# David-OConnor/molchanica

Hardware: AMD Instinct MI355X
Metric: MD atom-updates/sec (and steps/sec), 1M-atom solvated box (higher is better)
Workload: dtype f32

## Files before the change

### include/mdx.h

```cpp
#ifndef MDX_H
#define MDX_H

#include <stddef.h>
#include <stdint.h>

#ifdef __cplusplus
extern "C" {
#endif

#define MDX_OK       0
#define MDX_EPARAM  (-1)
#define MDX_EDEVICE (-2)
#define MDX_ENAN    (-3)
#define MDX_EOOM    (-4)

#define MDX_OVR_BONDED_DISABLED           0x1u
#define MDX_OVR_COULOMB_DISABLED          0x2u
#define MDX_OVR_LJ_DISABLED               0x4u
#define MDX_OVR_LONG_RANGE_RECIP_DISABLED 0x8u

#define MDX_ATOM_STATIC      0x1u
#define MDX_ATOM_BONDED_ONLY 0x2u
#define MDX_ATOM_GHOST       0x4u

// ... 122 lines not shown

int mdx_device_count(void);

const char* mdx_last_error(void);

void mdx_config_default(mdx_config* cfg);

int mdx_create(const mdx_system* sys, const mdx_config* cfg, int device, mdx_handle** out);
void mdx_destroy(mdx_handle* h);

int mdx_step(mdx_handle* h, float dt, const float* ext_forces, uint32_t n_steps);

int      mdx_set_position_restraints(mdx_handle* h, uint32_t n, const uint32_t* idx, const float* ref, const float* k,
                                     const float* flat_bottom);
uint32_t mdx_position_restraints_read(mdx_handle* h, uint32_t capacity, uint32_t* idx, float* ref, float* k, float* flat_bottom);
int      mdx_restraint_energy(mdx_handle* h, double* energy, double* virial);

int mdx_energy(mdx_handle* h, mdx_energies* out);

int mdx_single_point(const mdx_system* sys, const mdx_config* cfg, int device,
                     mdx_energies* out, float* forces_or_null);
void mdx_single_point_release(void);

int mdx_download(mdx_handle* h, int which, float* dst );
int mdx_upload(mdx_handle* h, int which, const float* src );
int mdx_upload_range(mdx_handle* h, int which, uint32_t first, uint32_t count, const float* src );

int mdx_set_box(mdx_handle* h, const float lo[3], const float hi[3]);
int mdx_rebuild_spatial_caches(mdx_handle* h);

uint64_t mdx_step_count(const mdx_handle* h);

int mdx_neighbor_list(mdx_handle* h, uint32_t* offsets , uint32_t* idx );

enum { MDX_HC_FLEXIBLE = 0, MDX_HC_SHAKE = 1, MDX_HC_LINEAR = 2 };
int mdx_set_hydrogen_constraint(mdx_handle* h, int kind, uint32_t lincs_order, uint32_t lincs_iter, float shake_tolerance);
const char* mdx_constraint_description(mdx_handle* h);

int mdx_profile(mdx_handle* h, int enable);
int mdx_get_stats(mdx_handle* h, mdx_stats* out);
int mdx_pair_launch_info(const mdx_handle* h, uint32_t out[24]);
int mdx_pair_body_info(const mdx_handle* h, uint32_t out[4]);
int mdx_fused_triad_info(const mdx_handle* h, uint32_t out[4]);
int mdx_get_skin(const mdx_handle* h, float* skin, int* tuning);

#define MDX_THERMOSTAT_NONE      0
#define MDX_THERMOSTAT_BERENDSEN 1
#define MDX_THERMOSTAT_CSVR      2

#define MDX_INTEGRATOR_VERLET_VELOCITY 0
#define MDX_INTEGRATOR_LEAPFROG        1
#define MDX_INTEGRATOR_LANGEVIN_MIDDLE 2
int mdx_set_integrator(mdx_handle* h, int kind, float gamma_per_ps, float temperature, uint64_t seed);

int mdx_set_alchemical_softcore(mdx_handle* h, float alpha, float sigma_min);
int mdx_configure_alchemical_window(mdx_handle* h, uint32_t mol_index, double lambda);

#define MDX_MAX_FOREIGN_LAMBDAS 32
int      mdx_set_foreign_lambdas(mdx_handle* h, uint32_t n, const double* lambdas);
int      mdx_foreign_energies(mdx_handle* h, double* du , uint32_t n);
uint32_t mdx_snapshot_foreign_count(const mdx_handle* h, uint32_t k);
int      mdx_snapshot_read_foreign(mdx_handle* h, uint32_t k, double* du, uint32_t n);

#define MDX_BAROSTAT_NONE      0
#define MDX_BAROSTAT_BERENDSEN 1
#define MDX_BAR_PER_KCAL_MOL_A3 69476.95
// ... 174 lines not shown
```

### molchanica_amd/csrc/mdx_api.hip

```cpp
#include "mdx_comm.h"
#include <algorithm>
#include <atomic>
#include <chrono>
#include <cfloat>
#include <cmath>
#include <cstring>
#include <dlfcn.h>
#include <mutex>
#include <unordered_map>

static thread_local std::string g_last_error;
void mdx_set_error(const std::string& s) { g_last_error = s; }

static inline unsigned div_up(unsigned a, unsigned b) { return (a + b - 1) / b; }
static bool cut_on(float rc) { return rc > 0.f && std::isfinite(rc); }
static uint32_t f2u(float f) { uint32_t u; std::memcpy(&u, &f, 4); return u; }
static float u2f(uint32_t u) { float f; std::memcpy(&f, &u, 4); return f; }

#define FAIL(code, msg) do { mdx_set_error(msg); return (code); } while (0)

template <typename T>
static int upload_vec(T** dptr, const std::vector<T>& v, hipStream_t st) {
    if (*dptr) { (void)hipFree(*dptr); *dptr = nullptr; }
    HIP_TRY(hipMalloc((void**)dptr, std::max<size_t>(sizeof(T) * v.size(), 16)));
// ... 1526 lines not shown
                              h->d.slot_of, h->d.posq, (float4*)d_out4,
                              flag_word >= 0 ? &h->d.ctl->disp2[flag_word] : nullptr);
    HIP_TRY(hipGetLastError());
    return MDX_OK;
}

extern "C" int mdx_unpack_positions(mdx_handle* h, const uint32_t* d_gid, uint32_t n, const float* d_in4,
                                    const float* d_shift4, int32_t flag_word) {
    if (!h || (n && (!d_gid || !d_in4)) || flag_word > (int32_t)MDX_MAX_CHUNK + 1) FAIL(MDX_EPARAM, "bad argument");
    if (!h->in_slot_space) FAIL(MDX_EPARAM, "spatial caches not built");
    const bool dual = h->dual_on && h->chunk_s >= 0;
    if (n) hipLaunchKernelGGL(unpack_pos_kernel, dim3(div_up(n, 256)), dim3(256), 0, h->stream, n, d_gid,
                              h->d.slot_of, h->d.posq, (const float4*)d_in4, (const float4*)d_shift4,
                              flag_word >= 0 ? &h->d.ctl->disp2[flag_word] : nullptr,
                              dual ? h->d.ref : nullptr,
                              dual ? (mdx_dd_split_now(h) ? &h->d.ctl->prune_ghost[h->chunk_s + 1]
                                                                                                      : &h->d.ctl->prune[h->chunk_s + 1]) : nullptr,
                              0.5f * h->inner_skin * (1.0f - 1.0e-4f),
                              h->dd ? h->box_hi[0] - h->box_lo[0] : 0.f, h->dd ? h->box_hi[1] - h->box_lo[1] : 0.f,
                              h->dd ? h->box_hi[2] - h->box_lo[2] : 0.f, (dual && h->path_split) ? h->d.path : nullptr);
    HIP_TRY(hipGetLastError());
    h->forces_valid = false;
    if (!dual) h->moved_outside = true;
    return MDX_OK;
}

extern "C" void* mdx_stream(mdx_handle* h) { return h ? (void*)h->stream : nullptr; }
extern "C" int mdx_debug_half_stats(mdx_handle* h, unsigned long long out[6]) {
    HIP_TRY(hipStreamSynchronize(h->stream));
    HIP_TRY(hipMemcpy(out, h->d.inner_count + MDX_EPART, sizeof(unsigned long long) * 6, hipMemcpyDeviceToHost));
    return MDX_OK;
}

static int posre_install(mdx_handle* h) {
    DeviceState& d = h->d;
    hipStream_t st = h->stream;
    const uint32_t N = h->N, R_old = h->n_roles, n = h->n_posre;
    std::vector<uint32_t> off_old(N + 1);
    std::vector<RoleRec> rec_old(R_old);
    std::vector<float4> prm(h->n_prm_base);
    HIP_TRY(hipMemcpyAsync(off_old.data(), d.role_off_o, sizeof(uint32_t) * (N + 1), hipMemcpyDeviceToHost, st));
    if (R_old) HIP_TRY(hipMemcpyAsync(rec_old.data(), d.role_rec_o, sizeof(RoleRec) * R_old, hipMemcpyDeviceToHost, st));
    if (!prm.empty()) HIP_TRY(hipMemcpyAsync(prm.data(), d.role_prm, sizeof(float4) * prm.size(), hipMemcpyDeviceToHost, st));
    HIP_TRY(hipStreamSynchronize(st));
    if ((size_t)h->n_prm_base + n >= ((size_t)1 << 24)) FAIL(MDX_EPARAM, "more than 16.7 M distinct bonded parameter sets with the restraints");
    std::vector<uint32_t> which(N, MDX_INVALID);
    for (uint32_t k = 0; k < n; ++k) which[h->posre_idx[k]] = k;
    std::vector<uint32_t> off(N + 1, 0);
    std::vector<RoleRec> rec;
    rec.reserve((size_t)R_old + n);
    for (uint32_t i = 0; i < N; ++i) {
        for (uint32_t k = off_old[i]; k < off_old[i + 1]; ++k)
            if ((rec_old[k].meta & 0xFu) != ROLE_POSRE) rec.push_back(rec_old[k]);
        if (which[i] != MDX_INVALID) {
            const uint32_t k = which[i];
            RoleRec r{};
            r.p[0] = i; r.p[1] = 0u; r.p[2] = f2u(h->posre_b[k]);
            r.meta = ROLE_POSRE | ((h->n_prm_base + k) << 8);
            rec.push_back(r);
        }
        off[i + 1] = (uint32_t)rec.size();
    }
    for (uint32_t k = 0; k < n; ++k)
        prm.push_back(make_float4(h->posre_ref[3 * k], h->posre_ref[3 * k + 1], h->posre_ref[3 * k + 2], h->posre_k[k]));
    const uint32_t R = (uint32_t)rec.size();
    h->n_roles = R;
// ... 77 lines not shown
```

### molchanica_amd/csrc/mdx_grid.hip

```cpp
#include "mdx_internal.h"
#include <atomic>
#include <chrono>
#include <algorithm>
#include <cfloat>
#include <cmath>

#define WAVE_LDS_SYNC()                                      \
    do {                                                     \
        __builtin_amdgcn_fence(__ATOMIC_SEQ_CST, "workgroup"); \
        __builtin_amdgcn_wave_barrier();                     \
    } while (0)

static inline unsigned div_up(unsigned a, unsigned b) { return (a + b - 1) / b; }

constexpr int SCAN_THREADS = 256;
constexpr int SCAN_ITEMS = 8;
constexpr int SCAN_TILE = SCAN_THREADS * SCAN_ITEMS;

template <int THREADS>
__device__ __forceinline__ uint32_t block_exclusive_scan(uint32_t v, uint32_t* s_wave , uint32_t* total) {
    const int lane = threadIdx.x & 63, wave = threadIdx.x >> 6;
    uint32_t inc = v;
#pragma unroll
    for (int d = 1; d < 64; d <<= 1) {
// ... 745 lines not shown
                const uint32_t sp = spc[q];
                if (sp == MDX_INVALID) continue;
#pragma unroll
                for (int e = 0; e < 8; ++e)
                    if (jcs[e] == (sp >> 3)) m &= ~(1ull << (8 * e + (sp & 7)));
            }
            for (uint32_t k = eb + LB_SPC; k < ee; ++k) {
                uint32_t sp = a.slot_of[a.excl_idx[k]];
                if (sp == MDX_INVALID) continue;
#pragma unroll
                for (int e = 0; e < 8; ++e)
                    if (jcs[e] == (sp >> 3)) m &= ~(1ull << (8 * e + (sp & 7)));
            }
        }
        if (a.mask_layout == 2) {
            const int ii = lane & 7, jj = lane >> 3;
            unsigned long long mq = 0ull;
#pragma unroll
            for (int ci = 0; ci < 8; ++ci) {
                const unsigned long long mp = __shfl(m, ci * 8 + ii);
#pragma unroll
                for (int e = 0; e < 8; ++e) mq |= ((mp >> (8 * e + jj)) & 1ull) << (8 * e + ci);
            }
            m = mq;
        }
        a.masks[(size_t)(mbase + c) * 64 + lane] = m;
    }
}

#ifndef PRUNE_TRIES
#define PRUNE_TRIES 1
#endif
struct PruneInner { uint2* entries_in; uint32_t* inner_nch; float rin2; WptRule rule; };
template <bool INNER>
__global__ __launch_bounds__(256) void prune_list_kernel(uint32_t T, float r2, float shx, float shy, float shz,
                                                         const float4* __restrict__ posq, ListCounts* __restrict__ counts,
                                                         const uint32_t* __restrict__ entry_off, uint2* __restrict__ entries,
                                                         uint32_t null_cluster, unsigned long long* __restrict__ pair_count,
                                                         const uint32_t* __restrict__ rb_ctl, uint32_t* __restrict__ tile_int,
                                                         const uint8_t* __restrict__ cl_kind, PruneInner pin) {
    __shared__ float4 s_j[4][64];
    const int lane = threadIdx.x & 63, wave = __builtin_amdgcn_readfirstlane(threadIdx.x >> 6);
    uint32_t first_ghost_cluster = 0xFFFFFFFFu;
    if (rb_ctl) {
        T = __builtin_amdgcn_readfirstlane(rb_ctl[0]); null_cluster = T * MDX_CL_PER_TILE;
        first_ghost_cluster = __builtin_amdgcn_readfirstlane(rb_ctl[1]) * MDX_CL_PER_TILE;
    }
    const bool inner_on = INNER && mdx_wpt_rule(pin.rule, T) == 1;
    bool ghost_hit = false;
    const uint32_t per_xcd = gridDim.x >> 3;
    const uint32_t t = MDX_XCD_SWIZZLE ? ((blockIdx.x & 7u) * per_xcd + (blockIdx.x >> 3)) * 4 + wave : blockIdx.x * 4 + wave;
    if (t >= T) return;
    const int ii = lane & 7, jj = lane >> 3;
    float xi[8], yi[8], zi[8];
#pragma unroll
    for (int ci = 0; ci < 8; ++ci) {
        const float4 p = posq[(size_t)t * MDX_TILE + ci * MDX_CLUSTER + ii];
        xi[ci] = p.x; yi[ci] = p.y; zi[ci] = p.z;
    }
    constexpr int NTRY = INNER ? 0 : PRUNE_TRIES;
    constexpr int TI[6] = {0, 7, 3, 0, 7, 4}, TJ[6] = {0, 7, 4, 7, 0, 3};
    float4 rep[NTRY ? NTRY : 1];
#pragma unroll
    for (int k = 0; k < NTRY; ++k) rep[k] = posq[(size_t)t * MDX_TILE + (lane & 7) * MDX_CLUSTER + TI[k]];
    uint32_t ilj = 0xFFu, iq = 0xFFu;
    if (cl_kind) {
        const uint32_t k = lane < MDX_CL_PER_TILE ? cl_kind[(size_t)t * MDX_CL_PER_TILE + lane] : 0u;
        ilj = (uint32_t)__ballot((k & 1u) != 0u) & 0xFFu; iq = (uint32_t)__ballot((k & 2u) != 0u) & 0xFFu;
    }
    const ListCounts cnt = counts[t];
    const uint32_t e0 = entry_off[t], nmc = cnt.n_masked >> 3, nchunks = (cnt.n_masked + cnt.n_plain) >> 3;
    uint32_t kept = 0, wcur = 0;
    uint32_t wcur_in = 0;
    uint2 ent_n = make_uint2(null_cluster, 13u), ent_nn = make_uint2(null_cluster, 13u);
    float4 pj_n = make_float4(0.f, 0.f, 0.f, 0.f);
    if (nchunks) { ent_n = entries[e0 + (lane >> 3)]; pj_n = posq[(size_t)ent_n.x * MDX_CLUSTER + (lane & 7)]; }
    if (nchunks > 1) ent_nn = entries[e0 + 8 + (lane >> 3)];
    for (uint32_t c = 0; c < nchunks; ++c) {
        const uint2 ent = ent_n;
        float4 pj = pj_n;
        if (c + 1 < nchunks) {
            ent_n = ent_nn;
            pj_n = posq[(size_t)ent_n.x * MDX_CLUSTER + (lane & 7)];
            if (c + 2 < nchunks) ent_nn = entries[e0 + (c + 2) * 8 + (lane >> 3)];
        }
        const uint32_t code = ent.y & 31u;
        pj.x += (float)((int)(code % 3u) - 1) * shx;
        pj.y += (float)((int)((code / 3u) % 3u) - 1) * shy;
        pj.z += (float)((int)(code / 9u) - 1) * shz;
        s_j[wave][lane] = pj;
        __builtin_amdgcn_fence(__ATOMIC_SEQ_CST, "workgroup"); __builtin_amdgcn_wave_barrier();
        uint32_t newy = ent.y;
        if (cl_kind) {
            const uint32_t kj = ent.x < null_cluster ? cl_kind[ent.x] : 0u;
            newy = (ent.y & 0xFFu) | (ent.y & ((((kj & 1u) ? ilj : 0u) | ((kj & 2u) ? iq : 0u)) << 8));
        }
        const uint32_t y_in = newy;
        uint32_t newy_in = newy & 0xFFu;
        unsigned long long acc = 0ull;
#pragma unroll
        for (int k = 0; k < NTRY; ++k) {
            const float4 q = s_j[wave][(lane & ~7) + TJ[k]];
            const float dx = rep[k].x - q.x, dy = rep[k].y - q.y, dz = rep[k].z - q.z;
            acc |= __ballot(dx * dx + dy * dy + dz * dz < r2);
        }
#pragma unroll 2
        for (int e = 0; e < 8; ++e) {
            const float4 q = s_j[wave][e * 8 + jj];
            const uint32_t y = __builtin_amdgcn_readlane(y_in, e * 8);
            const uint32_t sure = (uint32_t)(acc >> (e * 8)) & 0xFFu;
            uint32_t any = sure, anyin = 0u;
#pragma unroll
            for (int ci = 0; ci < 8; ++ci) {
                if (!(((y >> 8) & ~sure) & (1u << ci))) continue;
                const float dx = xi[ci] - q.x, dy = yi[ci] - q.y, dz = zi[ci] - q.z;
                const float d2 = dx * dx + dy * dy + dz * dz;
                const bool hit = __ballot(d2 < r2) != 0ull;
                any |= (hit ? 1u : 0u) << ci;
                if (INNER && hit) anyin |= (__ballot(d2 < pin.rin2) != 0ull ? 1u : 0u) << ci;
            }
            const uint32_t im = (y >> 8) & any;
            kept += __popc(im & 0xFFu);
            if ((lane >> 3) == e) newy = (y & 0xFFu) | ((im & 0xFFu) << 8);
            if (INNER && (lane >> 3) == e) newy_in = (y & 0xFFu) | ((((y >> 8) & anyin) & 0xFFu) << 8);
        }
        __builtin_amdgcn_fence(__ATOMIC_SEQ_CST, "workgroup"); __builtin_amdgcn_wave_barrier();
        ghost_hit |= ((newy >> 8) & 0xFFu) != 0u && ent.x >= first_ghost_cluster && ent.x < null_cluster;
        if (c < nmc) {
            if ((lane & 7) == 0 && newy != ent.y) entries[e0 + c * 8 + (lane >> 3)].y = newy;
            if (inner_on && (lane & 7) == 0) pin.entries_in[e0 + c * 8 + (lane >> 3)] = make_uint2(ent.x, newy_in);
        } else {
            const bool alive = (lane & 7) == 0 && ((newy >> 8) & 0xFFu) != 0u;
            const unsigned long long bal = __ballot(alive);
            if (alive) {
                const uint32_t rank = __popcll(bal & ((1ull << lane) - 1ull));
                entries[e0 + cnt.n_masked + wcur + rank] = make_uint2(ent.x, newy);
            }
            wcur += __popcll(bal);
            if (inner_on) {
                const bool alive_in = (lane & 7) == 0 && ((newy_in >> 8) & 0xFFu) != 0u;
                const unsigned long long bin = __ballot(alive_in);
                if (alive_in) pin.entries_in[e0 + cnt.n_masked + wcur_in + __popcll(bin & ((1ull << lane) - 1ull))] = make_uint2(ent.x, newy_in);
                wcur_in += __popcll(bin);
            }
        }
    }
    const uint32_t np_pad = (wcur + 7u) & ~7u;
    if (lane < (int)(np_pad - wcur)) entries[e0 + cnt.n_masked + wcur + lane] = make_uint2(null_cluster, 13u);
    if (inner_on) {
        const uint32_t nin_pad = (wcur_in + 7u) & ~7u;
        if (lane < (int)(nin_pad - wcur_in)) pin.entries_in[e0 + cnt.n_masked + wcur_in + lane] = make_uint2(null_cluster, 13u);
        if (lane < 8) pin.inner_nch[(size_t)t * 8 + lane] = nmc + (nin_pad >> 3);
    }
    const bool any_ghost = __any(ghost_hit);
    if (lane == 0) {
        counts[t].n_plain = np_pad;
        if (kept) atomicAdd(pc_slot(pair_count, t, 1), (unsigned long long)kept);
        if (tile_int) tile_int[t] = (!any_ghost && t * MDX_CL_PER_TILE < first_ghost_cluster) ? 1u : 0u;
    }
}

template <int W>
__global__ __launch_bounds__(W * 64) void prune_list_mw_kernel(uint32_t T, float r2, float shx, float shy, float shz,
                                                               const float4* __restrict__ posq, ListCounts* __restrict__ counts,
                                                               const uint32_t* __restrict__ entry_off, uint2* __restrict__ entries,
                                                               uint32_t null_cluster, unsigned long long* __restrict__ pair_count,
                                                               const uint32_t* __restrict__ rb_ctl, uint32_t* __restrict__ tile_int,
                                                               const uint8_t* __restrict__ cl_kind) {
    __shared__ float4 s_j[W][64];
    __shared__ uint32_t s_ghost;
    const int lane = threadIdx.x & 63, wave = __builtin_amdgcn_readfirstlane(threadIdx.x >> 6);
    uint32_t first_ghost_cluster = 0xFFFFFFFFu;
    if (rb_ctl) {
        T = __builtin_amdgcn_readfirstlane(rb_ctl[0]); null_cluster = T * MDX_CL_PER_TILE;
        first_ghost_cluster = __builtin_amdgcn_readfirstlane(rb_ctl[1]) * MDX_CL_PER_TILE;
    }
    const uint32_t t = blockIdx.x;
    if (t >= T) return;
    if (threadIdx.x == 0) s_ghost = 0u;
    if (tile_int) __syncthreads();
    bool ghost_hit = false;
    const int ii = lane & 7, jj = lane >> 3;
    float xi[8], yi[8], zi[8];
#pragma unroll
    for (int ci = 0; ci < 8; ++ci) {
        const float4 p = posq[(size_t)t * MDX_TILE + ci * MDX_CLUSTER + ii];
        xi[ci] = p.x; yi[ci] = p.y; zi[ci] = p.z;
    }
    const float4 rep = posq[(size_t)t * MDX_TILE + (lane & 7) * MDX_CLUSTER];
    uint32_t ilj = 0xFFu, iq = 0xFFu;
    if (cl_kind) {
        const uint32_t k = lane < MDX_CL_PER_TILE ? cl_kind[(size_t)t * MDX_CL_PER_TILE + lane] : 0u;
// ... 511 lines not shown
    }
    if (a.tile_order) {
        const uint32_t n_int = lpt_counting_sort(T, a.counts, 0u, a.tile_int, a.tile_order, s_sort);
        if (threadIdx.x == 0) s_nint = n_int;
    }
    if (threadIdx.x < 64) {
        const unsigned long long c = a.cursors[(size_t)threadIdx.x * 16];
        uint32_t e = (uint32_t)c, m = (uint32_t)(c >> 32);
        unsigned long long pa = a.pair_count[(size_t)threadIdx.x * PC_STRIDE], pb = a.pair_count[(size_t)threadIdx.x * PC_STRIDE + 1];
#pragma unroll
        for (int k = 32; k > 0; k >>= 1) { e += __shfl_xor(e, k); m += __shfl_xor(m, k); pa += __shfl_xor(pa, k); pb += __shfl_xor(pb, k); }
        if (threadIdx.x == 0) {
            a.pair_count[PC_TOTAL] = pa; a.pair_count[PC_TOTAL + 1] = pb;
            a.rb_ctl[RB_N_INT] = s_nint;
            a.host[0] = T; a.host[1] = a.rb_ctl[RB_T_OWN]; a.host[2] = a.rb_ctl[RB_NONFINITE]; a.host[3] = s_nint;
            for (int k = 0; k < 4; ++k) a.host[4 + k] = a.flags[k];
            a.host[8] = e; a.host[9] = m;
            a.host[10] = (uint32_t)pa; a.host[11] = (uint32_t)(pa >> 32); a.host[12] = (uint32_t)pb; a.host[13] = (uint32_t)(pb >> 32);
            a.rb_ctl[RB_NONFINITE] = 0u;
            __threadfence_system();
            a.host[31] = a.seq;
        }
    }
}


struct RebuildKnobs {
    bool fused;
    bool two_pass;
    bool exact_prune;
    int inner_mode;
    uint32_t mw_below;
    bool list_debug;
};
constexpr uint32_t PRUNE_MW_BELOW_FUSED = 12000u, PRUNE_MW_BELOW_UNFUSED = 2048u;
static const RebuildKnobs& rebuild_knobs() {
    static const RebuildKnobs k = [] {
        auto env = [](const char* name) { const char* e = std::getenv(name); return e ? e : ""; };
        RebuildKnobs r;
        r.fused = env("MDX_REBUILD_FUSED")[0] != '0';
        r.two_pass = env("MDX_LIST_TWO_PASS")[0] == '1';
        r.exact_prune = env("MDX_EXACT_PRUNE")[0] != '0';
        const char in = env("MDX_REBUILD_INNER")[0];
        r.inner_mode = in == '0' ? 0 : (in == '2' ? 2 : 1);
        const char* const mw = std::getenv("MDX_PRUNE_MW_BELOW");
        r.mw_below = mw ? (uint32_t)std::atoi(mw) : PRUNE_MW_BELOW_FUSED;
        r.list_debug = std::getenv("MDX_LIST_DEBUG") != nullptr;
        return r;
    }();
    return k;
}

struct RebuildResult { uint32_t E = 0, MC = 0; unsigned long long npairs = 0; bool ordered = false, classified = false, inner_built = false; };

struct TileOrderPlan { bool lpt, grouped, split; };
static TileOrderPlan tile_order_plan(const mdx_handle* h, uint32_t T) {
    static const int lpt_env = [] { const char* e = std::getenv("MDX_TILE_LPT"); return e ? (e[0] == '0' ? 0 : (e[0] == '2' ? 2 : 1)) : -1; }();
    const bool decomposed = h->dd || h->n_local != h->N;
    TileOrderPlan p;
    p.lpt = (lpt_env >= 0 ? lpt_env >= 1 : (decomposed || T >= 512u)) && mdx_nb_variant(h) >= 2;
    p.grouped = lpt_env >= 0 ? lpt_env == 2 : !decomposed;
    p.split = h->want_tile_split && mdx_nb_variant(h) >= 2;
    return p;
}

static bool list_is_pruned(const mdx_handle* h) { return !std::isinf(h->r_list) && mdx_nb_variant(h) >= 2; }

static float next_inner_skin(const mdx_handle* h) { return h->inner_skin_auto > 0.f ? h->inner_skin_auto : c_inner_skin(h->cfg); }
static bool dual_list_wanted(const mdx_handle* h, float inner_skin) {
    return !h->dual_auto_off && mdx_nb_half(h) && list_is_pruned(h) && inner_skin > 0.f && inner_skin < h->cfg.skin &&
           (h->n_vsites == 0 || h->vsites_convex);
}

static int list_flags_error(uint32_t f) {
    if (f & 1u) { mdx_set_error("exclusion table overflow while building the pair list"); return MDX_EPARAM; }
    if (f & 8u) { mdx_set_error("a constrained / virtual-site atom is missing from the local atom set"); return MDX_EPARAM; }
    if (f & 2u) { mdx_set_error("exclusion table overflow while building the pair list"); return MDX_EPARAM; }
    if (f & 4u) { mdx_set_error("a bonded partner of an owned atom is missing from the local atom set (halo too thin)"); return MDX_EPARAM; }
    return MDX_OK;
}
// ... 43 lines not shown
    a->cursors = reinterpret_cast<unsigned long long*>(h->d.list_cursors);
    a->n_regions = 1;
    while (a->n_regions < (uint32_t)LB_REGIONS && a->n_regions * 128u <= a->T) a->n_regions <<= 1;
    a->region_cap_e = (uint32_t)(std::min<uint64_t>(h->cap_entries, 0xFFFFFFFFull) / a->n_regions) & ~7u;
    a->region_cap_m = h->cap_mchunks / a->n_regions;
}

static void launch_single_pass(mdx_handle* h, ListArgs* a) {
    DeviceState& d = h->d;
    size_list_regions(h, a);
    a->list_grid = (div_up(a->T, LB_WAVES) + 7u) & ~7u;
    uint32_t rf_blocks = 0;
    if (h->n_roles) {
        a->rf_S = (a->T + 1) * MDX_TILE; a->rf_role_off_o = d.role_off_o; a->rf_rec_o = d.role_rec_o; a->rf_role_off_s = d.role_off_s;
        a->rf_rec_s = d.role_rec_s; a->rf_lflag = d.lflag; a->rf_tri_o = d.tri_o; a->rf_tri_s = d.tri_s;
        rf_blocks = div_up(a->rf_S, LB_WAVES * 64);
    }
    if (h->grid.npop > 1) hipLaunchKernelGGL((build_list_kernel<LB_SINGLE, LB_PLAIN_DD>), dim3(a->list_grid + rf_blocks), dim3(LB_WAVES * 64), 0, h->stream, *a);
    else hipLaunchKernelGGL(build_list_kernel<LB_SINGLE>, dim3(a->list_grid + rf_blocks), dim3(LB_WAVES * 64), 0, h->stream, *a);
}

static bool launch_exact_prune(mdx_handle* h, const ListArgs& a, uint32_t mw_below, const uint32_t* rb_ctl, uint32_t* tint, const PruneInner* inner) {
    DeviceState& d = h->d;
    hipStream_t st = h->stream;
    if (!a.T) return false;
    const float r2 = a.r_build * a.r_build;
    const float shx = h->per[0] ? h->box_hi[0] - h->box_lo[0] : 0.f, shy = h->per[1] ? h->box_hi[1] - h->box_lo[1] : 0.f,
                shz = h->per[2] ? h->box_hi[2] - h->box_lo[2] : 0.f;
    const uint8_t* const kinds = h->kind_split ? d.cl_kind : nullptr;
    const dim3 one_wave_grid((div_up(a.T, 4) + 7u) & ~7u);
    if (a.T < mw_below)
        hipLaunchKernelGGL(prune_list_mw_kernel<8>, dim3(a.T), dim3(512), 0, st, a.T, r2, shx, shy, shz, d.posq, d.list_counts,
                           d.entry_off, d.entries, a.null_cluster, d.pair_count, rb_ctl, tint, kinds);
    else if (inner)
        hipLaunchKernelGGL(prune_list_kernel<true>, one_wave_grid, dim3(256), 0, st, a.T, r2, shx, shy, shz,
                           d.posq, d.list_counts, d.entry_off, d.entries, a.null_cluster, d.pair_count, rb_ctl, tint, kinds, *inner);
    else
        hipLaunchKernelGGL(prune_list_kernel<false>, one_wave_grid, dim3(256), 0, st, a.T, r2, shx, shy, shz,
                           d.posq, d.list_counts, d.entry_off, d.entries, a.null_cluster, d.pair_count, rb_ctl, tint, kinds, PruneInner{});
    return inner && a.T >= mw_below;
}

static int rebuild_fast(mdx_handle* h, RebuildResult* res, bool* fell_back) {
    DeviceState& d = h->d;
    hipStream_t st = h->stream;
    const uint32_t N = h->n_local;
    const GridParams g = h->grid;
    const RebuildKnobs& knobs = rebuild_knobs();
    *fell_back = false;
    if (!d.rb_ctl) { ALLOC(d.rb_ctl, RB_WORDS); HIP_TRY(hipMemsetAsync(d.rb_ctl, 0, sizeof(uint32_t) * RB_WORDS, st)); }
    if (!d.pair_count) ALLOC(d.pair_count, PC_TOTAL + 2);
    if (!d.list_cursors) ALLOC(d.list_cursors, LB_REGIONS * 32 + 2);
    MDX_TRY(alloc_readback(h));
    if (!h->cell_count_clean) { HIP_TRY(hipMemsetAsync(d.cell_count, 0, sizeof(uint32_t) * ((size_t)h->ncells + 1), st)); h->cell_count_clean = true; }
    if (!h->slot_of_clean) { HIP_TRY(hipMemsetAsync(d.slot_of, 0xFF, sizeof(uint32_t) * (size_t)h->N, st)); h->slot_of_clean = true; }
    const uint32_t T_bound = N / MDX_TILE + h->ncol + 1;
    if (T_bound + 1 > h->cap_tiles) { *fell_back = true; return MDX_OK; }
    const TileOrderPlan plan = tile_order_plan(h, T_bound);
    const bool prune = list_is_pruned(h) && knobs.exact_prune;
    const bool classify_here = plan.split && plan.lpt && g.npop > 1 && prune;
    if (plan.lpt && (!d.tile_lpt || d.cap_tile_lpt < T_bound)) { d.cap_tile_lpt = h->cap_tiles + 1; ALLOC(d.tile_lpt, d.cap_tile_lpt); }
    if (classify_here && (!d.tile_bnd || h->cap_tile_split < T_bound + 1)) {
        h->cap_tile_split = h->cap_tiles + 1;
        ALLOC(d.tile_bnd, h->cap_tile_split); ALLOC(d.tile_scan, h->cap_tile_split); ALLOC(d.tile_order, h->cap_tile_split);
    }

    if (h->in_slot_space)
        hipLaunchKernelGGL(rb_prep_kernel<true>, dim3(div_up(N, 256)), dim3(256), 0, st, N, g, d.gid, d.slot_of, d.posq, d.vel, d.pos_orig,
                           d.vel_orig, d.lflag, d.cell_of, d.sorted_orig, d.cell_count, d.rb_ctl + RB_NONFINITE);
    else
        hipLaunchKernelGGL(rb_prep_kernel<false>, dim3(div_up(N, 256)), dim3(256), 0, st, N, g, d.gid, d.slot_of, d.posq, d.vel, d.pos_orig,
                           d.vel_orig, d.lflag, d.cell_of, d.sorted_orig, d.cell_count, d.rb_ctl + RB_NONFINITE);
// ... 374 lines not shown
```

### molchanica_amd/md_state.py

```python
from __future__ import annotations

import ctypes as C
import os

import numpy as np

from ._abi import (CCommDiag, CFlexOpts, CHBond, CConfig, CEnergies, CLUSTER_MAX_PERMS, CLUSTER_MAX_POSES, CLUSTER_POSES_ARGTYPES, CRefineOpts,
                   CSearchOpts, CStats, CSystem, FLEX_DIHEDRALS, FORCE, FUSED_TRIAD_INFO_ARGTYPES, POSE_RMSD_ARGTYPES,
                   MDX_EDEVICE, MDX_ENAN, MDX_EOOM, MDX_EPARAM, MDX_OK, POS, POSE_MAX_ATOMS, POSE_MAX_TORSIONS, VEL, MdConfig, MdSystem)

_HERE = os.path.dirname(os.path.abspath(__file__))
LIB_PATH = os.environ.get("MDX_LIB") or os.path.join(_HERE, "libmdx.so")


class ParamError(ValueError):
    """The reference's `ParamError { descrip }` (src/md/mod.rs:967)."""


class DeviceError(RuntimeError):
    """HIP/device failure (MDX_EDEVICE / MDX_EOOM); the reference degrades to its CPU path here
    (src/util.rs:1072-1119) — this library has none and says so loudly."""


class BlowUpError(FloatingPointError):
# ... 8 lines not shown
def load_library():
    global _lib
    if _lib is not None:
        return _lib
    if not os.path.exists(LIB_PATH):
        raise ImportError(
            f"{LIB_PATH} not found: the HIP extension is not built. Run "
            f"`python -c 'import __graft_entry__ as g; g.build()'` (no CPU fallback exists).")
    try:
        import torch
    except ImportError:
        pass
    lib = C.CDLL(LIB_PATH)
    H = C.c_void_p
    lib.mdx_device_count.restype = C.c_int
    lib.mdx_last_error.restype = C.c_char_p
    lib.mdx_config_default.argtypes = [C.POINTER(CConfig)]
    lib.mdx_create.argtypes = [C.POINTER(CSystem), C.POINTER(CConfig), C.c_int, C.POINTER(H)]
    lib.mdx_destroy.argtypes = [H]
    lib.mdx_destroy.restype = None
    lib.mdx_step.argtypes = [H, C.c_float, _fp, C.c_uint32]
    lib.mdx_energy.argtypes = [H, C.POINTER(CEnergies)]
    lib.mdx_single_point.argtypes = [C.POINTER(CSystem), C.POINTER(CConfig), C.c_int,
                                     C.POINTER(CEnergies), _fp]
    lib.mdx_download.argtypes = [H, C.c_int, _fp]
    lib.mdx_upload.argtypes = [H, C.c_int, _fp]
    lib.mdx_upload_range.argtypes = [H, C.c_int, C.c_uint32, C.c_uint32, _fp]
    lib.mdx_set_box.argtypes = [H, C.c_float * 3, C.c_float * 3]
    lib.mdx_shrink_cell_towards.argtypes = [H, C.c_float * 3, C.c_float * 3, C.c_float, C.POINTER(C.c_int)]
    lib.mdx_rebuild_spatial_caches.argtypes = [H]
    lib.mdx_step_count.argtypes = [H]
    lib.mdx_step_count.restype = C.c_uint64
    lib.mdx_neighbor_list.argtypes = [H, _u32p, _u32p]
    lib.mdx_profile.argtypes = [H, C.c_int]
    lib.mdx_get_stats.argtypes = [H, C.POINTER(CStats)]
    lib.mdx_get_skin.argtypes = [H, _fp, C.POINTER(C.c_int)]
    lib.mdx_pair_launch_info.argtypes = [H, _u32p]
    lib.mdx_pair_body_info.argtypes = [H, _u32p]
    lib.mdx_fused_triad_info.argtypes = FUSED_TRIAD_INFO_ARGTYPES
    lib.mdx_minimize_energy.argtypes = [H, C.c_uint32, _fp, C.c_float, C.POINTER(CEnergies), _u32p]
    lib.mdx_initialize_velocities.argtypes = [H, C.c_float, C.c_int, C.c_uint64]
    lib.mdx_set_thermostat.argtypes = [H, C.c_int, C.c_float, C.c_float, C.c_uint32, C.c_uint64]
    lib.mdx_set_barostat.argtypes = [H, C.c_int, C.c_float, C.c_float, C.c_float, C.c_uint32]
    lib.mdx_set_integrator.argtypes = [H, C.c_int, C.c_float, C.c_float, C.c_uint64]
    lib.mdx_configure_alchemical_window.argtypes = [H, C.c_uint32, C.c_double]
    lib.mdx_set_alchemical_softcore.argtypes = [H, C.c_float, C.c_float]
    lib.mdx_get_box.argtypes = [H, C.POINTER(C.c_float), C.POINTER(C.c_float)]
    lib.mdx_set_zero_com_drift.argtypes = [H, C.c_int]
    lib.mdx_set_snapshot_cadence.argtypes = [H, C.c_uint32, C.c_int]
    lib.mdx_set_energy_cadence.argtypes = [H, C.c_uint32]
    lib.mdx_snapshot_count.argtypes = [H]
    lib.mdx_snapshot_count.restype = C.c_uint32
    lib.mdx_snapshot_read.argtypes = [H, C.c_uint32, C.POINTER(C.c_double), C.POINTER(C.c_uint64),
                                      C.POINTER(CEnergies), _fp, _fp]
    lib.mdx_flush_snapshot_queues.argtypes = [H]
    lib.mdx_set_snapshot_handlers.argtypes = [H, _u32p]
    lib.mdx_snapshot_handler_mask.argtypes = [H, C.c_uint32]
    lib.mdx_snapshot_handler_mask.restype = C.c_uint32
    lib.mdx_snapshot_read_forces.argtypes = [H, C.c_uint32, _fp]
    lib.mdx_set_water_layout.argtypes = [H, C.c_uint32, C.c_uint32, C.c_uint32]
    lib.mdx_water_download.argtypes = [H, C.c_int, _fp, _fp, _fp, _fp]
    lib.mdx_set_hbond_detection.argtypes = [H, C.c_void_p, C.c_float, C.c_float]
    lib.mdx_snapshot_read_water.argtypes = [H, C.c_uint32, _fp, _fp, _fp]
    lib.mdx_snapshot_hbond_count.argtypes = [H, C.c_uint32]
    lib.mdx_snapshot_hbond_count.restype = C.c_uint32
    lib.mdx_snapshot_read_hbonds.argtypes = [H, C.c_uint32, C.POINTER(CHBond), C.c_uint32]
# ... 394 lines not shown
    def set_positions(self, pos):
        a = np.ascontiguousarray(pos, dtype=np.float32).reshape(self.n_atoms, 3)
        _check(load_library().mdx_upload(self._h, POS, a.ctypes.data_as(_fp)))

    def set_positions_range(self, first: int, pos):
        a = np.ascontiguousarray(pos, dtype=np.float32).reshape(-1, 3)
        _check(load_library().mdx_upload_range(self._h, POS, int(first), a.shape[0], a.ctypes.data_as(_fp)))

    def set_velocities(self, vel):
        a = np.ascontiguousarray(vel, dtype=np.float32).reshape(self.n_atoms, 3)
        _check(load_library().mdx_upload(self._h, VEL, a.ctypes.data_as(_fp)))

    def set_cell(self, lo, hi):
        _check(load_library().mdx_set_box(self._h, (C.c_float * 3)(*map(float, lo)),
                                          (C.c_float * 3)(*map(float, hi))))

    def shrink_cell_towards(self, target_lo, target_hi, shrink_per_step: float) -> bool:
        lo = (C.c_float * 3)(*[float(v) for v in target_lo]); hi = (C.c_float * 3)(*[float(v) for v in target_hi])
        out = C.c_int(0)
        _check(load_library().mdx_shrink_cell_towards(self._h, lo, hi, float(shrink_per_step), C.byref(out)))
        return bool(out.value)

    def rebuild_spatial_caches(self):
        _check(load_library().mdx_rebuild_spatial_caches(self._h))

    def neighbor_list(self):
        lib = load_library()
        off = np.zeros(self.n_atoms + 1, dtype=np.uint32)
        _check(lib.mdx_neighbor_list(self._h, off.ctypes.data_as(_u32p), None))
        idx = np.zeros(max(int(off[-1]), 1), dtype=np.uint32)
        _check(lib.mdx_neighbor_list(self._h, off.ctypes.data_as(_u32p), idx.ctypes.data_as(_u32p)))
        return off, idx[: int(off[-1])]

    def minimize_energy(self, max_iters: int, external_forces=None, f_tol: float = 0.0):
        ext = None
        if external_forces is not None:
            ext = np.ascontiguousarray(external_forces, dtype=np.float32).reshape(self.n_atoms, 3)
        e, it = CEnergies(), C.c_uint32(0)
        _check(load_library().mdx_minimize_energy(self._h, int(max_iters), None if ext is None else ext.ctypes.data_as(_fp),
                                                  float(f_tol), C.byref(e), C.byref(it)))
        return e.as_dict(), int(it.value)

    def initialize_velocities(self, temperature: float, zero_com_drift: bool = True, seed: int = 0):
        _check(load_library().mdx_initialize_velocities(self._h, float(temperature), int(zero_com_drift), int(seed)))

    def set_thermostat(self, kind: int, temp_target: float, tau_ps: float, every_n_steps: int = 10, seed: int = 0):
        _check(load_library().mdx_set_thermostat(self._h, int(kind), float(temp_target), float(tau_ps),
                                                 int(every_n_steps), int(seed)))

    def configure_alchemical_window(self, mol_index: int, lam: float):
        _check(load_library().mdx_configure_alchemical_window(self._h, int(mol_index), float(lam)))

    _foreign_lams = None

    def set_foreign_lambdas(self, lams):
        a = np.ascontiguousarray([] if lams is None else lams, dtype=np.float64).reshape(-1)
        _check(load_library().mdx_set_foreign_lambdas(self._h, a.shape[0], a.ctypes.data if a.shape[0] else None))
        self._foreign_lams = a.copy() if a.shape[0] else None

    def foreign_energies(self) -> np.ndarray:
        n = 0 if self._foreign_lams is None else self._foreign_lams.shape[0]
        out = np.zeros(max(n, 1), dtype=np.float64)
        _check(load_library().mdx_foreign_energies(self._h, out.ctypes.data, n))
        return out[:n]

    def set_alchemical_softcore(self, alpha: float = 0.5, sigma_min: float = 3.0):
# ... 308 lines not shown
```

Baseline: 2.289 billion.

## Replace per-pair ballots in list prune with packed hit bits and DPP wave-OR

```diff
diff --git a/include/mdx.h b/include/mdx.h
--- a/include/mdx.h
+++ b/include/mdx.h
@@ -178,6 +178,8 @@
 uint64_t mdx_step_count(const mdx_handle* h);
 
 int mdx_neighbor_list(mdx_handle* h, uint32_t* offsets , uint32_t* idx );
+
+int mdx_debug_pair_lists(mdx_handle* h, int which, uint32_t* dst, uint64_t capacity, uint64_t* n_out);
 
 enum { MDX_HC_FLEXIBLE = 0, MDX_HC_SHAKE = 1, MDX_HC_LINEAR = 2 };
 int mdx_set_hydrogen_constraint(mdx_handle* h, int kind, uint32_t lincs_order, uint32_t lincs_iter, float shake_tolerance);
diff --git a/molchanica_amd/csrc/mdx_api.hip b/molchanica_amd/csrc/mdx_api.hip
--- a/molchanica_amd/csrc/mdx_api.hip
+++ b/molchanica_amd/csrc/mdx_api.hip
@@ -1582,6 +1582,35 @@
     return MDX_OK;
 }
 
+extern "C" int mdx_debug_pair_lists(mdx_handle* h, int which, uint32_t* dst, uint64_t capacity, uint64_t* n_out) {
+    if (!h || !n_out || which < 0 || which > 5) FAIL(MDX_EPARAM, "bad argument");
+    if (!h->in_slot_space || !h->d.list_counts || !h->d.entry_off) FAIL(MDX_EPARAM, "spatial caches not built");
+    HIP_TRY(hipStreamSynchronize(h->stream));
+    const DeviceState& d = h->d;
+    const uint32_t T = h->T;
+    const void* src = nullptr;
+    uint64_t n = 0;
+    if (which == 0) { src = d.list_counts; n = 2ull * T; }
+    else if (which == 1) { src = d.entry_off; n = (uint64_t)T + 1; }
+    else if (which == 4) { src = d.inner_nch; n = d.inner_nch ? 8ull * T : 0; }
+    else if (which == 5) { src = d.orig_of; n = (uint64_t)T * MDX_TILE; }
+    else {
+        std::vector<ListCounts> cnt(T);
+        std::vector<uint32_t> off((size_t)T + 1);
+        if (T) HIP_TRY(hipMemcpy(cnt.data(), d.list_counts, sizeof(ListCounts) * T, hipMemcpyDeviceToHost));
+        HIP_TRY(hipMemcpy(off.data(), d.entry_off, sizeof(uint32_t) * ((size_t)T + 1), hipMemcpyDeviceToHost));
+        uint64_t ext = 0;
+        for (uint32_t t = 0; t < T; ++t) ext = std::max<uint64_t>(ext, (uint64_t)off[t] + cnt[t].n_masked + cnt[t].n_plain);
+        src = which == 2 ? d.entries : d.entries_in;
+        n = src ? 2 * ext : 0;
+    }
+    *n_out = n;
+    if (!dst) return MDX_OK;
+    if (capacity < n) FAIL(MDX_EPARAM, "capacity below the number of words");
+    if (n) HIP_TRY(hipMemcpy(dst, src, sizeof(uint32_t) * n, hipMemcpyDeviceToHost));
+    return MDX_OK;
+}
+
 static int posre_install(mdx_handle* h) {
     DeviceState& d = h->d;
     hipStream_t st = h->stream;
diff --git a/molchanica_amd/csrc/mdx_grid.hip b/molchanica_amd/csrc/mdx_grid.hip
--- a/molchanica_amd/csrc/mdx_grid.hip
+++ b/molchanica_amd/csrc/mdx_grid.hip
@@ -801,8 +801,16 @@
 #define PRUNE_TRIES 1
 #endif
 struct PruneInner { uint2* entries_in; uint32_t* inner_nch; float rin2; WptRule rule; };
-template <bool INNER>
-__global__ __launch_bounds__(256) void prune_list_kernel(uint32_t T, float r2, float shx, float shy, float shz,
+__device__ __forceinline__ uint32_t prune_or_wave(uint32_t v) {
+    v |= (uint32_t)__builtin_amdgcn_update_dpp(0, (int)v, 0xB1, 0xF, 0xF, true);
+    v |= (uint32_t)__builtin_amdgcn_update_dpp(0, (int)v, 0x4E, 0xF, 0xF, true);
+    v |= (uint32_t)__builtin_amdgcn_update_dpp(0, (int)v, 0x141, 0xF, 0xF, true);
+    v |= (uint32_t)__builtin_amdgcn_update_dpp(0, (int)v, 0x140, 0xF, 0xF, true);
+    return __builtin_amdgcn_readlane(v, 0) | __builtin_amdgcn_readlane(v, 16) | __builtin_amdgcn_readlane(v, 32) |
+           __builtin_amdgcn_readlane(v, 48);
+}
+template <bool INNER, int NTRY, bool HITBITS>
+__device__ __forceinline__ void prune_list_body(uint32_t T, float r2, float shx, float shy, float shz,
                                                          const float4* __restrict__ posq, ListCounts* __restrict__ counts,
                                                          const uint32_t* __restrict__ entry_off, uint2* __restrict__ entries,
                                                          uint32_t null_cluster, unsigned long long* __restrict__ pair_count,
@@ -827,11 +835,15 @@
         const float4 p = posq[(size_t)t * MDX_TILE + ci * MDX_CLUSTER + ii];
         xi[ci] = p.x; yi[ci] = p.y; zi[ci] = p.z;
     }
-    constexpr int NTRY = INNER ? 0 : PRUNE_TRIES;
     constexpr int TI[6] = {0, 7, 3, 0, 7, 4}, TJ[6] = {0, 7, 4, 7, 0, 3};
-    float4 rep[NTRY ? NTRY : 1];
-#pragma unroll
-    for (int k = 0; k < NTRY; ++k) rep[k] = posq[(size_t)t * MDX_TILE + (lane & 7) * MDX_CLUSTER + TI[k]];
+    __shared__ float4 s_i[HITBITS && NTRY ? 4 : 1][HITBITS && NTRY ? 64 : 1];
+    float4 rep[!HITBITS && NTRY ? NTRY : 1];
+    if constexpr (HITBITS && NTRY > 0) {
+        s_i[wave][lane] = posq[(size_t)t * MDX_TILE + lane];
+    } else {
+#pragma unroll
+        for (int k = 0; k < NTRY; ++k) rep[k] = posq[(size_t)t * MDX_TILE + (lane & 7) * MDX_CLUSTER + TI[k]];
+    }
     uint32_t ilj = 0xFFu, iq = 0xFFu;
     if (cl_kind) {
         const uint32_t k = lane < MDX_CL_PER_TILE ? cl_kind[(size_t)t * MDX_CL_PER_TILE + lane] : 0u;
@@ -841,6 +853,7 @@
     const uint32_t e0 = entry_off[t], nmc = cnt.n_masked >> 3, nchunks = (cnt.n_masked + cnt.n_plain) >> 3;
     uint32_t kept = 0, wcur = 0;
     uint32_t wcur_in = 0;
+    uint32_t kept_v = 0;
     uint2 ent_n = make_uint2(null_cluster, 13u), ent_nn = make_uint2(null_cluster, 13u);
     float4 pj_n = make_float4(0.f, 0.f, 0.f, 0.f);
     if (nchunks) { ent_n = entries[e0 + (lane >> 3)]; pj_n = posq[(size_t)ent_n.x * MDX_CLUSTER + (lane & 7)]; }
@@ -866,32 +879,85 @@
         }
         const uint32_t y_in = newy;
         uint32_t newy_in = newy & 0xFFu;
-        unsigned long long acc = 0ull;
-#pragma unroll
-        for (int k = 0; k < NTRY; ++k) {
-            const float4 q = s_j[wave][(lane & ~7) + TJ[k]];
-            const float dx = rep[k].x - q.x, dy = rep[k].y - q.y, dz = rep[k].z - q.z;
-            acc |= __ballot(dx * dx + dy * dy + dz * dz < r2);
-        }
+        if constexpr (!HITBITS) {
+            unsigned long long acc = 0ull;
+#pragma unroll
+            for (int k = 0; k < NTRY; ++k) {
+                const float4 q = s_j[wave][(lane & ~7) + TJ[k]];
+                const float dx = rep[k].x - q.x, dy = rep[k].y - q.y, dz = rep[k].z - q.z;
+                acc |= __ballot(dx * dx + dy * dy + dz * dz < r2);
+            }
 #pragma unroll 2
-        for (int e = 0; e < 8; ++e) {
-            const float4 q = s_j[wave][e * 8 + jj];
-            const uint32_t y = __builtin_amdgcn_readlane(y_in, e * 8);
-            const uint32_t sure = (uint32_t)(acc >> (e * 8)) & 0xFFu;
-            uint32_t any = sure, anyin = 0u;
-#pragma unroll
-            for (int ci = 0; ci < 8; ++ci) {
-                if (!(((y >> 8) & ~sure) & (1u << ci))) continue;
-                const float dx = xi[ci] - q.x, dy = yi[ci] - q.y, dz = zi[ci] - q.z;
-                const float d2 = dx * dx + dy * dy + dz * dz;
-                const bool hit = __ballot(d2 < r2) != 0ull;
-                any |= (hit ? 1u : 0u) << ci;
-                if (INNER && hit) anyin |= (__ballot(d2 < pin.rin2) != 0ull ? 1u : 0u) << ci;
+            for (int e = 0; e < 8; ++e) {
+                const float4 q = s_j[wave][e * 8 + jj];
+                const uint32_t y = __builtin_amdgcn_readlane(y_in, e * 8);
+                const uint32_t sure = (uint32_t)(acc >> (e * 8)) & 0xFFu;
+                uint32_t any = sure, anyin = 0u;
+#pragma unroll
+                for (int ci = 0; ci < 8; ++ci) {
+                    if (!(((y >> 8) & ~sure) & (1u << ci))) continue;
+                    const float dx = xi[ci] - q.x, dy = yi[ci] - q.y, dz = zi[ci] - q.z;
+                    const float d2 = dx * dx + dy * dy + dz * dz;
+                    const bool hit = __ballot(d2 < r2) != 0ull;
+                    any |= (hit ? 1u : 0u) << ci;
+                    if (INNER && hit) anyin |= (__ballot(d2 < pin.rin2) != 0ull ? 1u : 0u) << ci;
+                }
+                const uint32_t im = (y >> 8) & any;
+                kept += __popc(im & 0xFFu);
+                if ((lane >> 3) == e) newy = (y & 0xFFu) | ((im & 0xFFu) << 8);
+                if (INNER && (lane >> 3) == e) newy_in = (y & 0xFFu) | ((((y >> 8) & anyin) & 0xFFu) << 8);
             }
-            const uint32_t im = (y >> 8) & any;
-            kept += __popc(im & 0xFFu);
-            if ((lane >> 3) == e) newy = (y & 0xFFu) | ((im & 0xFFu) << 8);
-            if (INNER && (lane >> 3) == e) newy_in = (y & 0xFFu) | ((((y >> 8) & anyin) & 0xFFu) << 8);
+        } else {
+            unsigned long long sure_r = 0ull, sure_in = 0ull;
+            if constexpr (NTRY > 0) {
+                bool s_r = false, s_in = false;
+#pragma unroll
+                for (int k = 0; k < NTRY; ++k) {
+                    const float4 q = s_j[wave][(lane & ~7) + TJ[k]], p = s_i[wave][(lane & 7) * MDX_CLUSTER + TI[k]];
+                    const float dx = p.x - q.x, dy = p.y - q.y, dz = p.z - q.z;
+                    const float d2 = dx * dx + dy * dy + dz * dz;
+                    s_r |= d2 < r2;
+                    if (INNER) s_in |= d2 < pin.rin2;
+                }
+                sure_r = __ballot(s_r);
+                if (INNER) sure_in = __ballot(s_in);
+            }
+            uint32_t mine = 0u;
+#pragma unroll 1
+            for (int w = 0; w < 4; ++w) {
+                uint32_t hr = 0u, hi = 0u;
+#pragma unroll
+                for (int k = 0; k < 2; ++k) {
+                    const int e = w * 2 + k;
+                    const float4 q = s_j[wave][e * 8 + jj];
+                    const uint32_t y = __builtin_amdgcn_readlane(y_in, e * 8);
+                    const uint32_t open = (y >> 8) & ~(uint32_t)((INNER ? sure_in : sure_r) >> (e * 8)) & 0xFFu;
+#pragma unroll
+                    for (int ci = 0; ci < 8; ++ci) {
+                        if (!(open & (1u << ci))) continue;
+                        const float dx = xi[ci] - q.x, dy = yi[ci] - q.y, dz = zi[ci] - q.z;
+                        const float d2 = dx * dx + dy * dy + dz * dz;
+                        hr = __builtin_amdgcn_alignbit(hr, __float_as_uint(d2 - r2), 31);
+                        if (INNER) hi = __builtin_amdgcn_alignbit(hi, __float_as_uint(d2 - pin.rin2), 31);
+                    }
+                }
+                const uint32_t hb = prune_or_wave(INNER ? hr | (hi << 16) : hr);
+                if ((lane >> 4) == w) mine = hb;
+            }
+            const int le = lane >> 3, lci = lane & 7;
+            const uint32_t open_me = (y_in >> 8) & ~(uint32_t)((INNER ? sure_in : sure_r) >> (le * 8)) & 0xFFu;
+            const uint32_t open_next = (uint32_t)__builtin_amdgcn_update_dpp(0, (int)open_me, 0x128, 0xF, 0xF, true);
+            const uint32_t at = __popc(open_me >> (lci + 1)) + ((le & 1) ? 0u : __popc(open_next));
+            const bool tested = (open_me >> lci) & 1u;
+            const unsigned long long hit_r = __ballot(tested && ((mine >> at) & 1u)) | sure_r;
+            const unsigned long long hit_in = INNER ? __ballot(tested && ((mine >> (16 + at)) & 1u)) | sure_in : 0ull;
+            const uint32_t any = (uint32_t)(hit_r >> (le * 8)) & 0xFFu;
+            uint32_t anyin = (uint32_t)(hit_in >> (le * 8)) & 0xFFu;
+            anyin &= any;
+            const uint32_t im = (y_in >> 8) & any & 0xFFu;
+            newy = (y_in & 0xFFu) | (im << 8);
+            if (INNER) newy_in = (y_in & 0xFFu) | (((y_in >> 8) & anyin & 0xFFu) << 8);
+            kept_v += (lane & 7) == 0 ? __popc(im) : 0u;
         }
         __builtin_amdgcn_fence(__ATOMIC_SEQ_CST, "workgroup"); __builtin_amdgcn_wave_barrier();
         ghost_hit |= ((newy >> 8) & 0xFFu) != 0u && ent.x >= first_ghost_cluster && ent.x < null_cluster;
@@ -922,11 +988,31 @@
         if (lane < 8) pin.inner_nch[(size_t)t * 8 + lane] = nmc + (nin_pad >> 3);
     }
     const bool any_ghost = __any(ghost_hit);
+    if constexpr (HITBITS) {
+#pragma unroll
+        for (int k = 32; k > 0; k >>= 1) kept_v += __shfl_xor(kept_v, k);
+        kept = kept_v;
+    }
     if (lane == 0) {
         counts[t].n_plain = np_pad;
         if (kept) atomicAdd(pc_slot(pair_count, t, 1), (unsigned long long)kept);
         if (tile_int) tile_int[t] = (!any_ghost && t * MDX_CL_PER_TILE < first_ghost_cluster) ? 1u : 0u;
     }
+}
+
+#define PRUNE_LIST_PARAMS                                                                                                            \
+    uint32_t T, float r2, float shx, float shy, float shz, const float4* __restrict__ posq, ListCounts* __restrict__ counts,         \
+    const uint32_t* __restrict__ entry_off, uint2* __restrict__ entries, uint32_t null_cluster,                                      \
+    unsigned long long* __restrict__ pair_count, const uint32_t* __restrict__ rb_ctl, uint32_t* __restrict__ tile_int,                 \
+    const uint8_t* __restrict__ cl_kind, PruneInner pin
+#define PRUNE_LIST_ARGS T, r2, shx, shy, shz, posq, counts, entry_off, entries, null_cluster, pair_count, rb_ctl, tile_int, cl_kind, pin
+template <bool INNER>
+__global__ __launch_bounds__(256) void prune_list_kernel(PRUNE_LIST_PARAMS) {
+    prune_list_body<INNER, INNER ? 0 : PRUNE_TRIES, false>(PRUNE_LIST_ARGS);
+}
+template <bool INNER, int NTRY>
+__global__ __launch_bounds__(256) __attribute__((amdgpu_waves_per_eu(8))) void prune_list_hb_kernel(PRUNE_LIST_PARAMS) {
+    prune_list_body<INNER, NTRY, true>(PRUNE_LIST_ARGS);
 }
 
 template <int W>
@@ -1504,7 +1590,10 @@
     int inner_mode;
     uint32_t mw_below;
     bool list_debug;
+    bool prune_hitbits;
+    int prune_tries[2];
 };
+constexpr int PRUNE_HB_TRIES[2] = {1, 1};
 constexpr uint32_t PRUNE_MW_BELOW_FUSED = 12000u, PRUNE_MW_BELOW_UNFUSED = 2048u;
 static const RebuildKnobs& rebuild_knobs() {
     static const RebuildKnobs k = [] {
@@ -1518,6 +1607,9 @@
         const char* const mw = std::getenv("MDX_PRUNE_MW_BELOW");
         r.mw_below = mw ? (uint32_t)std::atoi(mw) : PRUNE_MW_BELOW_FUSED;
         r.list_debug = std::getenv("MDX_LIST_DEBUG") != nullptr;
+        r.prune_hitbits = env("MDX_PRUNE_HITBITS")[0] != '0';
+        const char* const tr[2] = {std::getenv("MDX_PRUNE_TRIES"), std::getenv("MDX_PRUNE_TRIES_INNER")};
+        for (int k = 0; k < 2; ++k) r.prune_tries[k] = tr[k] ? std::min(std::max(std::atoi(tr[k]), 0), 3) : PRUNE_HB_TRIES[k];
         return r;
     }();
     return k;
@@ -1627,12 +1719,19 @@
     if (a.T < mw_below)
         hipLaunchKernelGGL(prune_list_mw_kernel<8>, dim3(a.T), dim3(512), 0, st, a.T, r2, shx, shy, shz, d.posq, d.list_counts,
                            d.entry_off, d.entries, a.null_cluster, d.pair_count, rb_ctl, tint, kinds);
-    else if (inner)
-        hipLaunchKernelGGL(prune_list_kernel<true>, one_wave_grid, dim3(256), 0, st, a.T, r2, shx, shy, shz,
-                           d.posq, d.list_counts, d.entry_off, d.entries, a.null_cluster, d.pair_count, rb_ctl, tint, kinds, *inner);
-    else
-        hipLaunchKernelGGL(prune_list_kernel<false>, one_wave_grid, dim3(256), 0, st, a.T, r2, shx, shy, shz,
-                           d.posq, d.list_counts, d.entry_off, d.entries, a.null_cluster, d.pair_count, rb_ctl, tint, kinds, PruneInner{});
+    else {
+        using PruneFn = void (*)(uint32_t, float, float, float, float, const float4*, ListCounts*, const uint32_t*, uint2*, uint32_t,
+                                 unsigned long long*, const uint32_t*, uint32_t*, const uint8_t*, PruneInner);
+        static const PruneFn hitbits[2][4] = {
+            {prune_list_hb_kernel<false, 0>, prune_list_hb_kernel<false, 1>, prune_list_hb_kernel<false, 2>, prune_list_hb_kernel<false, 3>},
+            {prune_list_hb_kernel<true, 0>, prune_list_hb_kernel<true, 1>, prune_list_hb_kernel<true, 2>, prune_list_hb_kernel<true, 3>}};
+        static const PruneFn ballots[2] = {prune_list_kernel<false>, prune_list_kernel<true>};
+        const RebuildKnobs& knobs = rebuild_knobs();
+        const int fl = inner ? 1 : 0;
+        hipLaunchKernelGGL(knobs.prune_hitbits ? hitbits[fl][knobs.prune_tries[fl]] : ballots[fl], one_wave_grid, dim3(256), 0, st, a.T, r2,
+                           shx, shy, shz, d.posq, d.list_counts, d.entry_off, d.entries, a.null_cluster, d.pair_count, rb_ctl, tint, kinds,
+                           inner ? *inner : PruneInner{});
+    }
     return inner && a.T >= mw_below;
 }
 
diff --git a/molchanica_amd/md_state.py b/molchanica_amd/md_state.py
--- a/molchanica_amd/md_state.py
+++ b/molchanica_amd/md_state.py
@@ -64,6 +64,7 @@
     lib.mdx_step_count.argtypes = [H]
     lib.mdx_step_count.restype = C.c_uint64
     lib.mdx_neighbor_list.argtypes = [H, _u32p, _u32p]
+    lib.mdx_debug_pair_lists.argtypes = [H, C.c_int, _u32p, C.c_uint64, C.POINTER(C.c_uint64)]
     lib.mdx_profile.argtypes = [H, C.c_int]
     lib.mdx_get_stats.argtypes = [H, C.POINTER(CStats)]
     lib.mdx_get_skin.argtypes = [H, _fp, C.POINTER(C.c_int)]
@@ -524,6 +525,22 @@
         _check(lib.mdx_neighbor_list(self._h, off.ctypes.data_as(_u32p), idx.ctypes.data_as(_u32p)))
         return off, idx[: int(off[-1])]
 
+    PAIR_LIST_ARRAYS = ("counts", "entry_off", "entries", "entries_in", "inner_nch", "orig_of")
+
+    def debug_pair_lists(self):
+        lib = load_library()
+        out = {}
+        for which, name in enumerate(self.PAIR_LIST_ARRAYS):
+            n = C.c_uint64(0)
+            _check(lib.mdx_debug_pair_lists(self._h, which, None, 0, C.byref(n)))
+            a = np.zeros(int(n.value), dtype=np.uint32)
+            if a.size:
+                _check(lib.mdx_debug_pair_lists(self._h, which, a.ctypes.data_as(_u32p), a.size, C.byref(n)))
+            out[name] = a
+        for name, w in (("counts", 2), ("entries", 2), ("entries_in", 2), ("inner_nch", 8), ("orig_of", 64)):
+            out[name] = out[name].reshape(-1, w)
+        return out
+
     def minimize_energy(self, max_iters: int, external_forces=None, f_tol: float = 0.0):
         ext = None
         if external_forces is not None:
```

New measurement: 2.312 billion, median of 6. +1.0%, better.
